# Gadersd/whisper-burn

Hardware: NVIDIA H100
Metric: audio-seconds/sec (higher is better)
Workload: dtype f32 (fp16-exact weights, fp32 activations/accumulate)

## Files before the change

whisper-burn_b200/csrc/decoder4.cu:

```cuda
#include <cooperative_groups.h>

#include "dec_common.cuh"

namespace cg = cooperative_groups;

namespace wb {

namespace {

#ifndef D4_ASYNC
#define D4_ASYNC 1
#endif
#define D4_EXCHANGE(IDX, RXBYTES, SEND, PF)                  \
    do {                                                     \
        WB_FINE();                                           \
        __syncthreads();                                     \
        WB_FINE();                                           \
        SEND();                                              \
        WB_FINE();                                           \
        if (D4_ASYNC) {                                      \
            PF();                                            \
            WB_FINE();                                       \
            xwait(xbar + (IDX), (RXBYTES), lc & 1u);         \
        } else {                                             \
            cluster_arrive();                                \
            PF();                                            \
            WB_FINE();                                       \
            cluster_wait();                                  \
        }                                                    \
    } while (0)
#ifndef D4_FINE
#define D4_FINE 0
#endif
#if D4_FINE
#define WB_FINE() WB_TRACE()
#else
#define WB_FINE() do { } while (0)
#endif

constexpr int CS = 16;
constexpr int LG_NBUF = 3;
constexpr int LG_RB = 8;
constexpr int KV_STG = 4;
#ifndef D4_L2_CKV_KEEP
#define D4_L2_CKV_KEEP 0
#endif
__device__ __forceinline__ uint64_t ckv_policy() { return D4_L2_CKV_KEEP ? l2_policy_evict_last() : l2_policy_evict_first(); }

__device__ __forceinline__ void cluster_arrive() { asm volatile("barrier.cluster.arrive.release.aligned;" ::: "memory"); }
__device__ __forceinline__ void cluster_wait() { asm volatile("barrier.cluster.wait.acquire.aligned;" ::: "memory"); }

template <int NR>
struct RowBias {
    float bias[NR];
    float bias_own;
};
template <int NR, int VPL>
struct RowRegs : RowBias<NR> {
    uint4 v[NR][VPL];
};

template <int NR>
__device__ __forceinline__ void load_bias(const float* __restrict__ bias, int row0, int step, RowBias<NR>& r) {
    const int lane = threadIdx.x & 31;
#pragma unroll
    for (int i = 0; i < NR; ++i) r.bias[i] = __ldg(bias + row0 + i * step);
    r.bias_own = __ldg(bias + row0 + min(lane >> 1, NR - 1) * step);
}
template <int NR, int VPL>
__device__ __forceinline__ void load_rows(const __half* __restrict__ W, const float* __restrict__ bias, int K, int row0, int step,
                                          RowRegs<NR, VPL>& r, uint64_t pol) {
    const int lane = threadIdx.x & 31, nv = K / 8;
    load_bias<NR>(bias, row0, step, r);
#pragma unroll
    for (int i = 0; i < NR; ++i) {
        const uint4* p = reinterpret_cast<const uint4*>(W + (int64_t)(row0 + i * step) * K);
#pragma unroll
        for (int j = 0; j < VPL; ++j) {
            const int v = j * 32 + lane;
            r.v[i][j] = v < nv ? ldg_l2(p + v, pol) : make_uint4(0, 0, 0, 0);
        }
    }
}
template <int NR>
__device__ __forceinline__ float warp_reduce_owner(const float (&acc)[NR]) {
    const int lane = threadIdx.x & 31;
    float v8[8], v4[4], v2[2];
    {
        const bool up = lane & 16;
#pragma unroll
        for (int i = 0; i < 8; ++i) {
            const float lo = i < NR ? acc[i] : 0.0f, hi = i + 8 < NR ? acc[i + 8] : 0.0f;
            const float recv = __shfl_xor_sync(0xffffffffu, up ? lo : hi, 16);
            v8[i] = (up ? hi : lo) + recv;
        }
    }
    {
        const bool up = lane & 8;
#pragma unroll
        for (int i = 0; i < 4; ++i) {
            const float recv = __shfl_xor_sync(0xffffffffu, up ? v8[i] : v8[i + 4], 8);
            v4[i] = (up ? v8[i + 4] : v8[i]) + recv;
        }
    }
    {
        const bool up = lane & 4;
#pragma unroll
        for (int i = 0; i < 2; ++i) {
            const float recv = __shfl_xor_sync(0xffffffffu, up ? v4[i] : v4[i + 2], 4);
            v2[i] = (up ? v4[i + 2] : v4[i]) + recv;
        }
    }
    const bool up = lane & 2;
    float v = (up ? v2[1] : v2[0]) + __shfl_xor_sync(0xffffffffu, up ? v2[0] : v2[1], 2);
    v += __shfl_xor_sync(0xffffffffu, v, 1);
    return v;
}

template <int NR, int VPL, bool REDUCE, typename WV>
__device__ __forceinline__ void dot_rows(WV&& wv, const float* xs, int K, float (&acc)[NR]) {
    const int lane = threadIdx.x & 31, nv = K / 8;
#pragma unroll
    for (int i = 0; i < NR; ++i) acc[i] = 0.0f;
#pragma unroll
    for (int j = 0; j < VPL; ++j) {
        const int v = j * 32 + lane;
        if (v < nv) {
            const float4 x0 = *reinterpret_cast<const float4*>(xs + v * 8);
            const float4 x1 = *reinterpret_cast<const float4*>(xs + v * 8 + 4);
#pragma unroll
            for (int i = 0; i < NR; ++i) {
                float w[8];
                cvt8(wv(i, j), w);
                float a = acc[i];
                a = fmaf(w[0], x0.x, a); a = fmaf(w[1], x0.y, a); a = fmaf(w[2], x0.z, a); a = fmaf(w[3], x0.w, a);
                a = fmaf(w[4], x1.x, a); a = fmaf(w[5], x1.y, a); a = fmaf(w[6], x1.z, a); a = fmaf(w[7], x1.w, a);
                acc[i] = a;
            }
        }
    }
    if constexpr (REDUCE) {
#pragma unroll
        for (int i = 0; i < NR; ++i) acc[i] = warp_sum(acc[i]);
    }
}
template <int NR, int VPL, bool REDUCE = true>
__device__ __forceinline__ void dot_rows1(const RowRegs<NR, VPL>& r, const float* xs, int K, float (&acc)[NR]) {
    dot_rows<NR, VPL, REDUCE>([&](int i, int j) { return r.v[i][j]; }, xs, K, acc);
}
template <int NR, int VPL, bool REDUCE = true>
__device__ __forceinline__ void dot_rows1s(const uint8_t* ws, const float* xs, int K, float (&acc)[NR]) {
    const int lane = threadIdx.x & 31, nv = K / 8;
    const uint4* w = reinterpret_cast<const uint4*>(ws) + (threadIdx.x >> 5) * nv;
    dot_rows<NR, VPL, REDUCE>([&](int i, int j) { return w[i * NW * nv + j * 32 + lane]; }, xs, K, acc);
}
__device__ __forceinline__ void bulk_rows(uint8_t* dst, const __half* W, int K, int row0, int n, uint64_t* bar) {
    const uint32_t bytes = (uint32_t)n * K * 2;
    fence_proxy_async();
    mbar_expect_tx(bar, bytes);
    bulk_g2s_l2(dst, W + (int64_t)row0 * K, bytes, bar, l2_policy_evict_last());
}

__device__ __forceinline__ void st_async_v4(uint32_t raddr, const float4& v, uint32_t rbar) {
    asm volatile("st.async.shared::cluster.mbarrier::complete_tx::bytes.v4.f32 [%0], {%1, %2, %3, %4}, [%5];" ::"r"(raddr), "f"(v.x),
                 "f"(v.y), "f"(v.z), "f"(v.w), "r"(rbar)
                 : "memory");
}
__device__ __forceinline__ void put16(cg::cluster_group& cl, float* dst, uint64_t* bar, int dest, const float4& v) {
#if D4_ASYNC
    st_async_v4(mapa_u32(smem_u32(dst), (uint32_t)dest), v, mapa_u32(smem_u32(bar), (uint32_t)dest));
#else
    *reinterpret_cast<float4*>(cl.map_shared_rank(dst, dest)) = v;
#endif
}
template <int CNT>
__device__ __forceinline__ void put_slice(cg::cluster_group& cl, const float* stage_s, float* dst_local, uint64_t* bar) {
    static_assert(CNT % 4 == 0, "slice must be a whole number of 16-byte vectors");
    constexpr int Q = CNT / 4;
    for (int i = threadIdx.x; i < CS * Q; i += NT) {
        const int dest = i / Q, q = i - dest * Q;
        put16(cl, dst_local + 4 * q, bar, dest, reinterpret_cast<const float4*>(stage_s)[q]);
    }
}
__device__ __forceinline__ void xwait(uint64_t* bar, uint32_t bytes, uint32_t parity) {
    if (threadIdx.x == 0) mbar_expect_tx(bar, bytes);
    const uint32_t mb = smem_u32(bar);
    uint32_t done = 0;
    int spins = 0;
    while (!done) {
        done = mbar_try_wait(mb, parity);
        if (!done && ++spins > (1 << 24)) __trap();
    }
}

template <int PF>
struct XRegs {
    float4 v[PF];
};
__device__ __forceinline__ float4 add4(const float4& a, const float4& b) {
    return make_float4(__fadd_rn(a.x, b.x), __fadd_rn(a.y, b.y), __fadd_rn(a.z, b.z), __fadd_rn(a.w, b.w));
}
template <int PF>
__device__ __forceinline__ void x_update(XRegs<PF>& x, const float* src_s, const float* d_s, float* dst_s) {
    const int lane = threadIdx.x & 31;
#pragma unroll
    for (int k = 0; k < PF; ++k)
        x.v[k] = add4(reinterpret_cast<const float4*>(src_s)[lane + 32 * k], reinterpret_cast<const float4*>(d_s)[lane + 32 * k]);
    if (dst_s != nullptr && threadIdx.x < 32) {
#pragma unroll
        for (int k = 0; k < PF; ++k) reinterpret_cast<float4*>(dst_s)[lane + 32 * k] = x.v[k];
    }
}
template <int D, int PF>
__device__ __forceinline__ void ln_fetch(float* lnp, const float* __restrict__ g, const float* __restrict__ b, uint64_t pol) {
    const int lane = threadIdx.x & 31;
#pragma unroll
    for (int k = 0; k < PF; ++k) {
        cp_async16_l2(lnp + 4 * (lane + 32 * k), g + 4 * (lane + 32 * k), pol);
        cp_async16_l2(lnp + D + 4 * (lane + 32 * k), b + 4 * (lane + 32 * k), pol);
    }
}
template <int D, int PF>
__device__ __forceinline__ void ln_warp(XRegs<PF>& x, const float* gb_s, float eps, int eps_outside, float* out_s) {
    const int lane = threadIdx.x & 31;
    cp_async_wait_all();
    float s = 0.0f;
#pragma unroll
    for (int k = 0; k < PF; ++k) s += (x.v[k].x + x.v[k].y) + (x.v[k].z + x.v[k].w);
    s = warp_sum(s);
    const float mean = __fdiv_rn(s, (float)D);
    float q = 0.0f;
#pragma unroll
    for (int k = 0; k < PF; ++k) {
        x.v[k].x = __fsub_rn(x.v[k].x, mean); x.v[k].y = __fsub_rn(x.v[k].y, mean);
        x.v[k].z = __fsub_rn(x.v[k].z, mean); x.v[k].w = __fsub_rn(x.v[k].w, mean);
        q = fmaf(x.v[k].x, x.v[k].x, q); q = fmaf(x.v[k].y, x.v[k].y, q);
        q = fmaf(x.v[k].z, x.v[k].z, q); q = fmaf(x.v[k].w, x.v[k].w, q);
    }
    q = warp_sum(q);
    const float var = __fdiv_rn(q, (float)D);
    const float den = eps_outside ? __fadd_rn(__fsqrt_rn(var), eps) : __fsqrt_rn(__fadd_rn(var, eps));
    const float rinv = __fdiv_rn(1.0f, den);
#pragma unroll
    for (int k = 0; k < PF; ++k) {
        const float4 g = reinterpret_cast<const float4*>(gb_s)[lane + 32 * k];
        const float4 b = reinterpret_cast<const float4*>(gb_s + D)[lane + 32 * k];
        reinterpret_cast<float4*>(out_s)[lane + 32 * k] =
            make_float4(fmaf(__fmul_rn(x.v[k].x, rinv), g.x, b.x), fmaf(__fmul_rn(x.v[k].y, rinv), g.y, b.y),
                        fmaf(__fmul_rn(x.v[k].z, rinv), g.z, b.z), fmaf(__fmul_rn(x.v[k].w, rinv), g.w, b.w));
    }
    __syncwarp();
}

template <int D, int RC, typename KVT>
__global__ void __launch_bounds__(NT, 1)
dec4_kernel(const DecArgs a) {
    extern __shared__ __align__(16) float sm[];
    cg::cluster_group cl = cg::this_cluster();
    constexpr int H = D / 64;
    constexpr int VPL = (D / 8 + 31) / 32;
    constexpr int VPL4 = (4 * D / 8 + 31) / 32;
    constexpr int NR_QKV = 3 * D / (CS * NW), NR_D = D / (CS * NW), NR_H = 4 * D / (CS * NW);
    const int L = a.L, V = a.V, R = a.R, t_max = a.t_max;
    const int tid = threadIdx.x, warp = tid >> 5, lane = tid & 31;
    const int rank = (int)cl.block_rank();
    const int row = blockIdx.x / CS;
    const bool active = row < R;

    float* lnp = sm + warp * 2 * D;
    float* qkv_s = sm + NW * 2 * D;
    float* att_s = qkv_s + 3 * D;
    float* dl_s = att_s + D;
    float* q2_s = dl_s + D;
    float* hid_s = q2_s + D;
    float* part_s = hid_s + 4 * D;
    float* wm = part_s + CS * 68;
    float* wl = wm + NW;
    float* wo = wl + NW;
    float* ao = wo + NW * 64;
    float* ML = ao + 64;
    constexpr int STG_N = 4 * D / CS > 68 ? 4 * D / CS : 68;
    float* stg_s = ML + 4;
    float* xb = stg_s + STG_N;
    float* xn_s = xb + 2 * D;
    float* red = xn_s + D;
    constexpr int RINGW = (LG_NBUF * LG_RB * D * 2 > KV_STG * 8 * 128 * 4) ? LG_NBUF * LG_RB * D * 2 : KV_STG * 8 * 128 * 4;
    constexpr int LG_PITCH = D * 2;
    uint8_t* ring = reinterpret_cast<uint8_t*>(red + NW * 4 * RC * 6);
    uint64_t* lg_bar = reinterpret_cast<uint64_t*>(ring + (size_t)NW * RINGW);
    uint64_t* kv_bar = lg_bar + NW * LG_NBUF;
    uint64_t* xbar = kv_bar + NW * KV_STG;
    uint64_t* wt_bar = xbar + 8;
    uint4* pl_hi = reinterpret_cast<uint4*>(wt_bar + 4);
    uint4* pl_lo = pl_hi + (D / 32) * 32;
    constexpr int QKV_B = 3 * D / CS * D * 2, W1_B = 4 * D / CS * D * 2, W2_B = D / CS * 4 * D * 2;
    constexpr int QKV_OFF = 0, W1_OFF = 0, W2_OFF = W1_OFF + W1_B;
    static_assert(W2_OFF + W2_B <= NW * RINGW, "W1 and W2 must fit the ring");
    static_assert(QKV_OFF + QKV_B <= W2_OFF, "the next layer's Wqkv arrives while W2 is read: no overlap");
    static_assert(QKV_B % 16 == 0 && W1_B % 16 == 0 && W2_B % 16 == 0 && W2_OFF % 16 == 0, "bulk copies move 16-byte units");
    if (lane == 0) {
        for (int j = 0; j < KV_STG; ++j) mbar_init(kv_bar + warp * KV_STG + j, 1);
        for (int j = 0; j < LG_NBUF; ++j) mbar_init(lg_bar + warp * LG_NBUF + j, 1);
        if (warp == 0) {
            for (int j = 0; j < 8; ++j) mbar_init(xbar + j, 1);
            for (int j = 0; j < 3; ++j) mbar_init(wt_bar + j, 1);
        }
        mbar_fence_init();
    }
    cl.sync();
    unsigned int lc = 0;
    unsigned int kv_count = 0;
    unsigned int lg_count = 0;
    unsigned int gen = 0;
    unsigned int lstep = 0;
    int tr_n = 0;
    const float scale = a.qk_scale;
    auto issue_qkv = [&](int l) {
        if (tid == 0) bulk_rows(ring + QKV_OFF, reinterpret_cast<const __half*>(a.layers[l].Wqkv), D, rank * (3 * D / CS), 3 * D / CS, wt_bar + 0);
    };
    auto demote = [&]() {
        const size_t gt = (size_t)blockIdx.x * NT + tid, gn = (size_t)gridDim.x * NT;
        for (int l = 0; l < L; ++l) {
            const DecLayer& W = a.layers[l];
            l2_demote(W.Wqkv, (size_t)3 * D * D * 2, gt, gn);
            l2_demote(W.Wo, (size_t)D * D * 2, gt, gn);
            l2_demote(W.Wcq, (size_t)D * D * 2, gt, gn);
            l2_demote(W.Wco, (size_t)D * D * 2, gt, gn);
            l2_demote(W.W1, (size_t)4 * D * D * 2, gt, gn);
            l2_demote(W.W2, (size_t)4 * D * D * 2, gt, gn);
            l2_demote(W.ln1_g, D * 4, gt, gn); l2_demote(W.ln1_b, D * 4, gt, gn); l2_demote(W.ln2_g, D * 4, gt, gn);
            l2_demote(W.ln2_b, D * 4, gt, gn); l2_demote(W.ln3_g, D * 4, gt, gn); l2_demote(W.ln3_b, D * 4, gt, gn);
        }
        l2_demote(a.lnf_g, D * 4, gt, gn);
        l2_demote(a.lnf_b, D * 4, gt, gn);
        const size_t kv_bytes = (size_t)L * a.Rmax * t_max * D * sizeof(KVT);
        l2_demote(a.kc, kv_bytes, gt, gn);
        l2_demote(a.vc, kv_bytes, gt, gn);
        if (D4_L2_CKV_KEEP) l2_demote(a.ckv, (size_t)L * a.Mcap * 2 * D * sizeof(KVT), gt, gn);
    };
    WB_TRACE();

    const __half* nullw = nullptr;
    (void)nullw;
    for (int step = 0; step < a.n_steps; ++step) {
        const int p = a.pos0 + step;
        const bool want_logits = p >= a.logits_from;
        constexpr int KH = D / 2, NCH = KH / 32;
        constexpr uint32_t BLKB = 16 * KH * 2;
        static_assert(LG_NBUF * LG_RB * D * 2 >= LG_NBUF * (int)BLKB, "ring slot too small");
        const __half* Et = reinterpret_cast<const __half*>(a.E_tiled);
        const int v_tiles = (V + 15) / 16;
        const int t0w = (int)blockIdx.x + (int)gridDim.x * warp, tstep = (int)gridDim.x * NW;
        const int my_tiles = t0w < v_tiles ? (v_tiles - t0w + tstep - 1) / tstep : 0;
        const int total = my_tiles * 2;
        auto tile_of = [&](int i) { return t0w + i * tstep; };
        uint8_t* wring = ring + (size_t)warp * RINGW;
        uint64_t* wbar = lg_bar + warp * LG_NBUF;
        auto issue = [&](int it) {
            if (it < total && lane == 0) {
                const int vt = tile_of(it >> 1);
                const int slot = (int)((lg_count + (unsigned int)it) % LG_NBUF);
                mbar_expect_tx(wbar + slot, BLKB);
                bulk_g2s_l2(wring + (size_t)slot * BLKB, Et + ((int64_t)vt * 2 + (it & 1)) * 16 * KH, BLKB, wbar + slot, l2_policy_evict_first());
            }
        };
        uint4* gpl_hi = reinterpret_cast<uint4*>(a.att_pl);
        uint4* gpl_lo = gpl_hi + (D / 32) * 32;
        if (want_logits && !active) {
#pragma unroll
            for (int j = 0; j < LG_NBUF; ++j) issue(j);
        }
        if (active) {
            const int tok = __ldcg(a.tokens + (int64_t)row * t_max + p);
            const int xh = rank % H, xci = rank / H;
            const int xnch = (CS - xh + H - 1) / H;
            const int xw = __ldcg(a.row_window + row);
            const int xT = a.win_T[xw];
            const int64_t xoff = a.win_row_off[xw] * (int64_t)(2 * D) + (int64_t)xh * xT * 128;
            const int sub = lane >> 2, l4 = lane & 3;
            const bool self_fast = p + 1 <= NW * 16;
            constexpr int PF = D / 128;
            static_assert(D % 128 == 0, "row must be a whole number of float4s per lane");
            int xsel = 0;
            XRegs<PF> x;
#pragma unroll
            for (int k = 0; k < PF; ++k)
                x.v[k] = add4(__ldg(reinterpret_cast<const float4*>(a.tok_emb + (int64_t)tok * D) + lane + 32 * k),
                              __ldg(reinterpret_cast<const float4*>(a.pos_emb + (int64_t)p * D) + lane + 32 * k));
            if (warp == 0) {
#pragma unroll
                for (int k = 0; k < PF; ++k) reinterpret_cast<float4*>(xb)[lane + 32 * k] = x.v[k];
            }
            RowBias<NR_QKV> b_qkv;
            load_bias<NR_QKV>(a.layers[0].bqkv, rank * (3 * D / CS) + warp, NW, b_qkv);
            if (step == 0) issue_qkv(0);
            if (step == 0) ln_fetch<D, PF>(lnp, a.layers[0].ln1_g, a.layers[0].ln1_b, l2_policy_evict_last());
            __syncthreads();
            for (int l = 0; l < L; ++l) {
                const DecLayer& W = a.layers[l];
                KVT* kcl = reinterpret_cast<KVT*>(a.kc) + (size_t)l * a.Rmax * t_max * D;
                KVT* vcl = reinterpret_cast<KVT*>(a.vc) + (size_t)l * a.Rmax * t_max * D;
                if (l > 0) {
                    x_update<PF>(x, xb + xsel * D, dl_s, xb + (xsel ^ 1) * D);
                    xsel ^= 1;
                }
                ln_warp<D, PF>(x, lnp, W.ln1_eps, a.eps_outside, xn_s);
                ln_fetch<D, PF>(lnp, W.ln2_g, W.ln2_b, l2_policy_evict_last());
                {
                    float acc[NR_QKV];
                    mbar_wait(wt_bar + 0, lc & 1u);
                    dot_rows1s<NR_QKV, VPL, false>(ring + QKV_OFF, xn_s, D, acc);
                    float mine = warp_reduce_owner<NR_QKV>(acc);
                    mine = __fadd_rn(mine, b_qkv.bias_own);
                    const int j = warp + (lane >> 1) * NW;
                    if (rank * (3 * D / CS) + j < 2 * D) mine = __fmul_rn(mine, scale);
                    if (!(lane & 1) && (lane >> 1) < NR_QKV) stg_s[j] = mine;
                }
                RowRegs<NR_D, VPL> w_o;
                constexpr int SNV = sizeof(KVT) == 4 ? 4 : 2;
                uint8_t* sring = ring + (size_t)warp * RINGW;
                auto pre_s2 = [&]() {
                    load_rows<NR_D, VPL>(reinterpret_cast<const __half*>(W.Wo), W.bo, D, rank * (D / CS) + warp, NW, w_o, l2_policy_evict_last());
                    if (rank < H && self_fast) {
#pragma unroll
                        for (int u = 0; u < 2; ++u) {
                            const int j = warp + NW * (u * 8 + sub);
                            if (j < p) {
                                const int64_t o = ((int64_t)row * t_max + j) * D + rank * 64 + l4 * 16;
#pragma unroll
                                for (int c = 0; c < SNV; ++c) {
                                    cp_async16_l2(sring + ((u * 2 + 0) * 4 + c) * 512 + lane * 16, reinterpret_cast<const uint4*>(kcl + o) + c, l2_policy_evict_last());
                                    cp_async16_l2(sring + ((u * 2 + 1) * 4 + c) * 512 + lane * 16, reinterpret_cast<const uint4*>(vcl + o) + c, l2_policy_evict_last());
                                }
                            }
                        }
                    }
                };
                auto send_s1 = [&]() {
                    put_slice<3 * D / CS>(cl, stg_s, qkv_s + rank * (3 * D / CS), xbar + 0);
                    if (tid < 3 * D / CS) {
                        const int n = rank * (3 * D / CS) + tid;
                        const float v = stg_s[tid];
                        if (n >= 2 * D) vcl[((int64_t)row * t_max + p) * D + (n - 2 * D)] = (KVT)v;
                        else if (n >= D) kcl[((int64_t)row * t_max + p) * D + (n - D)] = (KVT)v;
                    }
                };
                D4_EXCHANGE(0, 3 * D * 4, send_s1, pre_s2);
                if (D4_ASYNC && !self_fast) cl.sync();
                WB_TRACE();
                if (rank < H) {
                    const int h = rank;
                    if (self_fast) {
                        cp_async_wait_all();
                        float q[16];
#pragma unroll
                        for (int c = 0; c < 4; ++c) {
                            const float4 t4 = *reinterpret_cast<const float4*>(qkv_s + h * 64 + l4 * 16 + c * 4);
                            q[c * 4] = t4.x; q[c * 4 + 1] = t4.y; q[c * 4 + 2] = t4.z; q[c * 4 + 3] = t4.w;
                        }
                        AttnAcc A;
                        A.m = -INFINITY;
                        A.l = 0.0f;
#pragma unroll
                        for (int c = 0; c < 16; ++c) A.o[c] = 0.0f;
#pragma unroll
                        for (int u = 0; u < 2; ++u) {
                            const int j = warp + NW * (u * 8 + sub);
                            float4 skk[4], svv[4];
                            if (j < p) {
                                if constexpr (sizeof(KVT) == 4) {
#pragma unroll
                                    for (int c = 0; c < 4; ++c) {
                                        skk[c] = *reinterpret_cast<const float4*>(sring + ((u * 2 + 0) * 4 + c) * 512 + lane * 16);
                                        svv[c] = *reinterpret_cast<const float4*>(sring + ((u * 2 + 1) * 4 + c) * 512 + lane * 16);
                                    }
                                } else {
#pragma unroll
                                    for (int c = 0; c < 2; ++c) {
                                        float w8[8];
                                        cvt8(*reinterpret_cast<const uint4*>(sring + ((u * 2 + 0) * 4 + c) * 512 + lane * 16), w8);
                                        skk[2 * c] = make_float4(w8[0], w8[1], w8[2], w8[3]); skk[2 * c + 1] = make_float4(w8[4], w8[5], w8[6], w8[7]);
                                        cvt8(*reinterpret_cast<const uint4*>(sring + ((u * 2 + 1) * 4 + c) * 512 + lane * 16), w8);
                                        svv[2 * c] = make_float4(w8[0], w8[1], w8[2], w8[3]); svv[2 * c + 1] = make_float4(w8[4], w8[5], w8[6], w8[7]);
                                    }
                                }
                            } else {
#pragma unroll
                                for (int c = 0; c < 4; ++c) { skk[c] = make_float4(0.f, 0.f, 0.f, 0.f); svv[c] = skk[c]; }
                            }
                            if (j == p) {
#pragma unroll
                                for (int c = 0; c < 4; ++c) {
                                    float4 k4 = *reinterpret_cast<const float4*>(qkv_s + D + h * 64 + l4 * 16 + c * 4);
                                    float4 v4 = *reinterpret_cast<const float4*>(qkv_s + 2 * D + h * 64 + l4 * 16 + c * 4);
                                    if constexpr (sizeof(KVT) == 2) {
                                        k4 = make_float4((float)(KVT)k4.x, (float)(KVT)k4.y, (float)(KVT)k4.z, (float)(KVT)k4.w);
                                        v4 = make_float4((float)(KVT)v4.x, (float)(KVT)v4.y, (float)(KVT)v4.z, (float)(KVT)v4.w);
                                    }
                                    skk[c] = k4;
                                    svv[c] = v4;
                                }
                            }
                            attn_regs_step(q, skk, svv, j <= p, A);
                        }
                        attn_merge_subs(A);
                        attn_cta_tail(A, wm, wl, wo, ao, ML);
                    } else {
                        const KVT* kb = kcl + h * 64;
                        const KVT* vb = vcl + h * 64;
                        auto kp = [&](int j) { return kb + ((int64_t)row * t_max + j) * D; };
                        auto vp = [&](int j) { return vb + ((int64_t)row * t_max + j) * D; };
                        attn_cta(qkv_s + h * 64, p + 1, kp, vp, wm, wl, wo, ao, ML);
                    }
                }
                auto send_s2 = [&]() {
                    if (rank < H) {
                        const int dest = tid >> 4, q = tid & 15;
                        const float4 o4 = reinterpret_cast<const float4*>(ao)[q];
                        const float den = ML[1];
                        put16(cl, att_s + rank * 64 + 4 * q, xbar + 1, dest,
                              make_float4(__fdiv_rn(o4.x, den), __fdiv_rn(o4.y, den), __fdiv_rn(o4.z, den), __fdiv_rn(o4.w, den)));
                    }
                };
                auto pf_none = [&]() {};
                D4_EXCHANGE(1, D * 4, send_s2, pf_none);
                WB_TRACE();
                {
                    float acc[NR_D];
                    dot_rows1<NR_D, VPL>(w_o, att_s, D, acc);
                    WB_FINE();
                    if (lane == 0) {
#pragma unroll
                        for (int i = 0; i < NR_D; ++i) stg_s[warp + i * NW] = __fadd_rn(acc[i], w_o.bias[i]);
                    }
                }
                RowRegs<NR_D, VPL> w_cq;
                auto pre_s4 = [&]() {
                    load_rows<NR_D, VPL>(reinterpret_cast<const __half*>(W.Wcq), W.bcq, D, rank * (D / CS) + warp, NW, w_cq, l2_policy_evict_last());
                    fence_proxy_async();
                    attn_bulk_prefill<KV_STG, KVT, true>(reinterpret_cast<const KVT*>(a.ckv) + (size_t)l * a.Mcap * 2 * D + xoff, xT, xci * NW + warp,
                                                         xnch * NW, ring + (size_t)warp * RINGW, kv_bar + warp * KV_STG, kv_count, ckv_policy());
                };
                auto send_s3 = [&]() { put_slice<D / CS>(cl, stg_s, dl_s + rank * (D / CS), xbar + 2); };
                D4_EXCHANGE(2, D * 4, send_s3, pre_s4);
                WB_TRACE();
                x_update<PF>(x, xb + xsel * D, dl_s, xb + (xsel ^ 1) * D);
                xsel ^= 1;
                ln_warp<D, PF>(x, lnp, W.ln2_eps, a.eps_outside, xn_s);
                ln_fetch<D, PF>(lnp, W.ln3_g, W.ln3_b, l2_policy_evict_last());
                WB_FINE();
                {
                    float acc[NR_D];
                    dot_rows1<NR_D, VPL>(w_cq, xn_s, D, acc);
                    WB_FINE();
                    if (lane == 0) {
#pragma unroll
                        for (int i = 0; i < NR_D; ++i) stg_s[warp + i * NW] = __fmul_rn(__fadd_rn(acc[i], w_cq.bias[i]), scale);
                    }
                }
                RowRegs<NR_D, VPL> w_co;
                auto pre_s6 = [&]() { load_rows<NR_D, VPL>(reinterpret_cast<const __half*>(W.Wco), W.bco, D, rank * (D / CS) + warp, NW, w_co, l2_policy_evict_last()); };
                auto send_s4 = [&]() { put_slice<D / CS>(cl, stg_s, q2_s + rank * (D / CS), xbar + 3); };
                D4_EXCHANGE(3, D * 4, send_s4, pre_s6);
                WB_TRACE();
                {
                    const int h = xh, ci = xci, nch = xnch, T = xT;
                    const KVT* kbase = reinterpret_cast<const KVT*>(a.ckv) + (size_t)l * a.Mcap * 2 * D + xoff;
                    AttnAcc A;
                    attn_warp_bulk<KV_STG, KVT, true>(q2_s + h * 64, kbase, T, ci * NW + warp, nch * NW, 0, ring + (size_t)warp * RINGW,
                                                      kv_bar + warp * KV_STG, kv_count, A, true, ckv_policy());
                    if (lane < 4) {
#pragma unroll
                        for (int c = 0; c < 16; ++c) wo[warp * 64 + attn_bulk_dim<KVT>(lane, c)] = A.o[c];
                    }
                    if (lane == 0) { wm[warp] = A.m; wl[warp] = A.l; }
                    __syncthreads();
                    if (tid < 64) {
                        float M = -INFINITY;
#pragma unroll
                        for (int w2 = 0; w2 < NW; ++w2) M = fmaxf(M, wm[w2]);
                        float Ls = 0.0f, o = 0.0f;
#pragma unroll
                        for (int w2 = 0; w2 < NW; ++w2) {
                            const float m = wm[w2];
                            const float sc = m > -INFINITY ? expf(m - M) : 0.0f;
                            Ls += sc * wl[w2];
                            o += sc * wo[w2 * 64 + tid];
                        }
                        stg_s[4 + tid] = o;
                        if (tid < 4) stg_s[tid] = tid == 0 ? M : tid == 1 ? Ls : 0.0f;
                    }
                }
                auto send_s5 = [&]() { put_slice<68>(cl, stg_s, part_s + rank * 68, xbar + 4); };
                auto pre_mlp = [&]() {
                    if (tid == 0) {
                        bulk_rows(ring + W1_OFF, reinterpret_cast<const __half*>(W.W1), D, rank * (4 * D / CS), 4 * D / CS, wt_bar + 1);
                        bulk_rows(ring + W2_OFF, reinterpret_cast<const __half*>(W.W2), 4 * D, rank * (D / CS), D / CS, wt_bar + 2);
                    }
                };
                D4_EXCHANGE(4, CS * 68 * 4, send_s5, pre_mlp);
                WB_TRACE();
                for (int c = tid; c < D; c += NT) {
                    const int h = c / 64;
                    float M = -INFINITY;
                    for (int k = h; k < CS; k += H) M = fmaxf(M, part_s[k * 68]);
                    float den = 0.0f, num = 0.0f;
                    for (int k = h; k < CS; k += H) {
                        const float m = part_s[k * 68];
                        const float wgt = m > -INFINITY ? expf(m - M) : 0.0f;
                        den += wgt * part_s[k * 68 + 1];
                        num += wgt * part_s[k * 68 + 4 + (c & 63)];
                    }
                    att_s[c] = __fdiv_rn(num, den);
                }
                __syncthreads();
                {
                    float acc[NR_D];
                    dot_rows1<NR_D, VPL>(w_co, att_s, D, acc);
                    if (lane == 0) {
#pragma unroll
                        for (int i = 0; i < NR_D; ++i) stg_s[warp + i * NW] = __fadd_rn(acc[i], w_co.bias[i]);
                    }
                }
                RowBias<NR_H> b_1;
                auto pre_s7 = [&]() { load_bias<NR_H>(W.b1, rank * (4 * D / CS) + warp, NW, b_1); };
                auto send_s6 = [&]() { put_slice<D / CS>(cl, stg_s, dl_s + rank * (D / CS), xbar + 5); };
                D4_EXCHANGE(5, D * 4, send_s6, pre_s7);
                WB_TRACE();
                x_update<PF>(x, xb + xsel * D, dl_s, xb + (xsel ^ 1) * D);
                xsel ^= 1;
                ln_warp<D, PF>(x, lnp, W.ln3_eps, a.eps_outside, xn_s);
                if (l == L - 1 && want_logits && rank == 0 && warp == 0) {
                    ln_fetch<D, PF>(lnp, a.lnf_g, a.lnf_b, l2_policy_evict_last());
                } else {
                    const DecLayer& Wn = a.layers[l + 1 < L ? l + 1 : 0];
                    ln_fetch<D, PF>(lnp, Wn.ln1_g, Wn.ln1_b, l2_policy_evict_last());
                }
                WB_FINE();
                {
                    float acc[NR_H];
                    mbar_wait(wt_bar + 1, lc & 1u);
                    dot_rows1s<NR_H, VPL, false>(ring + W1_OFF, xn_s, D, acc);
                    float mine = warp_reduce_owner<NR_H>(acc);
                    mine = gelu_erf(__fadd_rn(mine, b_1.bias_own));
                    WB_FINE();
                    if (!(lane & 1) && (lane >> 1) < NR_H) stg_s[warp + (lane >> 1) * NW] = mine;
                }
                RowBias<NR_D> b_2;
                auto pre_s8 = [&]() {
                    load_bias<NR_D>(W.b2, rank * (D / CS) + warp, NW, b_2);
                    if (l + 1 < L) issue_qkv(l + 1);
                    else if (!want_logits && step + 1 < a.n_steps) issue_qkv(0);
                };
                auto send_s7 = [&]() { put_slice<4 * D / CS>(cl, stg_s, hid_s + rank * (4 * D / CS), xbar + 6); };
                D4_EXCHANGE(6, 4 * D * 4, send_s7, pre_s8);
                WB_TRACE();
                {
                    float acc[NR_D];
                    mbar_wait(wt_bar + 2, lc & 1u);
                    dot_rows1s<NR_D, VPL4>(ring + W2_OFF, hid_s, 4 * D, acc);
                    if (lane == 0) {
#pragma unroll
                        for (int i = 0; i < NR_D; ++i) stg_s[warp + i * NW] = __fadd_rn(acc[i], b_2.bias[i]);
                    }
                }
                auto pre_s1 = [&]() {
                    if (l + 1 < L) {
                        load_bias<NR_QKV>(a.layers[l + 1].bqkv, rank * (3 * D / CS) + warp, NW, b_qkv);
                    } else if (want_logits) {
                        fence_proxy_async();
#pragma unroll
                        for (int j = 0; j < LG_NBUF; ++j) issue(j);
                    }
                };
                auto send_s8 = [&]() { put_slice<D / CS>(cl, stg_s, dl_s + rank * (D / CS), xbar + 7); };
                D4_EXCHANGE(7, D * 4, send_s8, pre_s1);
                ++lc;
                WB_TRACE();
            }
            if (want_logits && rank == 0 && warp == 0) {
                x_update<PF>(x, xb + xsel * D, dl_s, nullptr);
                ln_warp<D, PF>(x, lnp, a.lnf_eps, a.eps_outside, xn_s);
#pragma unroll
                for (int k = 0; k < PF; ++k)
                    store_frag(gpl_hi, RC == 4 ? gpl_hi + 16 : gpl_lo, D / 32, row, 4 * (lane + 32 * k), reinterpret_cast<const float4*>(xn_s)[lane + 32 * k]);
                ln_fetch<D, PF>(lnp, a.layers[0].ln1_g, a.layers[0].ln1_b, l2_policy_evict_last());
            }
        }
        if (!want_logits) {
            if (D4_ASYNC && active) cl.sync();
            continue;
        }
        WB_TRACE();
        grid_sync(a.bar, gen);
        WB_TRACE();
        {
            const bool use_mask = SPECIAL_MASKED(a, p);
            const int eot_cap = a.loop_rules ? a.eot : -1;
            for (int i = tid; i < 2 * (D / 32) * 32; i += NT) cp_async16(pl_hi + i, gpl_hi + i);
            cp_async_wait_all();
            __syncthreads();
            WB_TRACE();
            const int g = lane >> 2, t = lane & 3;
            float m_run[2] = {-INFINITY, -INFINITY}, s_run[2] = {0.0f, 0.0f}, bv[2] = {-INFINITY, -INFINITY};
            int bi[2] = {INT_MAX, INT_MAX};
            float ah[4], al[4];
            unsigned int sp01 = 0;
#pragma unroll 1
            for (int it = 0; it < total; ++it) {
                const unsigned int cnt = lg_count + (unsigned int)it;
                const int slot = (int)(cnt % LG_NBUF);
                mbar_wait(wbar + slot, (cnt / LG_NBUF) & 1);
                const uint8_t* blk = wring + (size_t)slot * BLKB;
                const int half = it & 1;
                if (half == 0) {
#pragma unroll
                    for (int c = 0; c < 4; ++c) { ah[c] = 0.0f; al[c] = 0.0f; }
                    if (use_mask) {
                        const int n = tile_of(it >> 1) * 16 + g;
                        sp01 = (n < V ? ldg_l2(a.is_special + n, l2_policy_evict_first()) : 0u) | (n + 8 < V ? ldg_l2(a.is_special + n + 8, l2_policy_evict_first()) << 8 : 0u);
                    }
                }
#pragma unroll
                for (int c = 0; c < NCH; ++c) {
                    const uint4 a0 = *reinterpret_cast<const uint4*>(blk + (size_t)g * (KH * 2) + c * 64 + t * 16);
                    const uint4 a8 = *reinterpret_cast<const uint4*>(blk + (size_t)(g + 8) * (KH * 2) + c * 64 + t * 16);
                    const int chunk = half * NCH + c;
                    const uint4 bh = pl_hi[chunk * 32 + lane];
                    mma16816(ah, a0.x, a8.x, a0.y, a8.y, bh.x, bh.y);
                    mma16816(ah, a0.z, a8.z, a0.w, a8.w, bh.z, bh.w);
                    if constexpr (RC != 4) {
                        const uint4 bl = pl_lo[chunk * 32 + lane];
                        mma16816(al, a0.x, a8.x, a0.y, a8.y, bl.x, bl.y);
                        mma16816(al, a0.z, a8.z, a0.w, a8.w, bl.z, bl.w);
                    }
                }
                if (half == 1) {
                    const int n0 = tile_of(it >> 1) * 16;
#pragma unroll
                    for (int c = 0; c < 4; ++c) {
                        const int n = n0 + g + (c >> 1) * 8, e = c & 1;
                        if constexpr (RC == 4) al[c] = __shfl_xor_sync(0xffffffffu, ah[c], 2);
                        if (n < V && 2 * t + e < R) {
                            const float raw = hl_join(ah[c], al[c]);
                            const float v = (use_mask && ((sp01 >> ((c >> 1) * 8)) & 0xffu)) ? __fadd_rn(raw, -INFINITY) : raw;
                            if (v > -INFINITY) softmax_add(m_run[e], s_run[e], v);
                            if (cand_better(v, n, bv[e], bi[e])) { bv[e] = v; bi[e] = n; }
                            if (n == eot_cap) a.eot_logit[2 * t + e] = v;
                        }
                    }
                }
                __syncwarp();
                issue(it + LG_NBUF);
            }
            lg_count += (unsigned int)total;
            WB_TRACE();
#pragma unroll
            for (int e = 0; e < 2; ++e) {
#pragma unroll
                for (int off = 4; off < 32; off <<= 1) {
                    softmax_merge(m_run[e], s_run[e], __shfl_xor_sync(0xffffffffu, m_run[e], off), __shfl_xor_sync(0xffffffffu, s_run[e], off));
                    cand_xor(bv[e], bi[e], off);
                }
                if (g == 0) {
                    float* rec = red + (warp * 8 + 2 * t + e) * 4;
                    rec[0] = m_run[e]; rec[1] = s_run[e]; rec[2] = bv[e]; rec[3] = __int_as_float(bi[e]);
                }
            }
            __syncthreads();
            if (active && step + 1 < a.n_steps) issue_qkv(0);
            if (tid < R) fold_records_top1(a, red + tid * 4, NW, 8 * 4, (int64_t)blockIdx.x * R + tid);
        }
        WB_TRACE();
        ++lstep;
        __syncthreads();
        if (tid == 0) reinterpret_cast<int*>(ML)[2] = last_ticket(a.bar, lstep);
        __syncthreads();
        WB_TRACE();
        if (reinterpret_cast<int*>(ML)[2]) {
            __threadfence();
            for (int r = warp; r < R; r += NW) finish_row_top1<4>(a, r, p, gridDim.x);
            __syncthreads();
            if (tid == 0) release_flag(a.bar, lstep);
        }
        WB_TRACE();
        if (tid == 0) wait_flag(a.bar, lstep, 40000000000LL);
        __syncthreads();
        WB_TRACE();
        if (rows_open(a) == 0) {
            if (active && tid == 0 && step + 1 < a.n_steps) mbar_wait(wt_bar + 0, lc & 1u);
            if (blockIdx.x == 0 && tid == 0) decode_done(a, p + 1, 0, step + 1);
            demote();
            return;
        }
    }
    if (a.n_steps > 0 && a.pos0 + a.n_steps - 1 < a.logits_from) grid_sync(a.bar, gen);
    demote();
    if (blockIdx.x == 0 && tid == 0) decode_done(a, a.pos0 + a.n_steps, rows_open(a), a.n_steps);
}

template <int D, int RC>
constexpr size_t dec4_smem() {
    return sizeof(float) * ((size_t)(2 * NW + 13) * D + (4 * D / CS > 68 ? 4 * D / CS : 68) + CS * 68 + 2 * NW + NW * 64 + 64 + 4 + (size_t)NW * 4 * RC * 6 + 16) +
           (size_t)NW * std::max(LG_NBUF * LG_RB * D * 2, KV_STG * 8 * 128 * 4) + NW * LG_NBUF * 8 + NW * KV_STG * 8 + 8 * 8 + 4 * 8 + (size_t)2 * (D / 32) * 32 * 16 + 16;
}
static_assert(dec4_smem<384, 8>() <= 227 * 1024 && dec4_smem<384, 4>() <= 227 * 1024, "dec4_kernel exceeds the shared memory of an sm_90 CTA");

template <int D, int RC, typename KVT>
bool launch4_t(const DecArgs& a, cudaStream_t st) {
    const void* k = (const void*)dec4_kernel<D, RC, KVT>;
    const size_t smem = dec4_smem<D, RC>();
    static ClusterLaunch cl;
    const int n_cl = std::min(cl.capacity(k, CS, NT, smem, "dec4"), 8);
    if (n_cl < 1 || a.R > n_cl) return false;
    void* args[] = {(void*)&a};
    cl.launch(k, CS, n_cl, NT, smem, args, st, "dec4");
    return true;
}

}

bool launch_dec4(const DecArgs& a, bool w_half, cudaStream_t st) {
    if (!w_half || a.R > 8 || a.R < 1 || a.k != 1 || !a.greedy || a.use_cur_tok || a.anc != nullptr || a.logits_out != nullptr) return false;
    if (a.H * 64 != a.d || a.H > CS || a.E_tiled == nullptr) return false;
#define WB_D4(DD)                                                                                         \
    do {                                                                                                  \
        if (a.kv_half) return a.R <= 4 ? launch4_t<DD, 4, __half>(a, st) : launch4_t<DD, 8, __half>(a, st); \
        return a.R <= 4 ? launch4_t<DD, 4, float>(a, st) : launch4_t<DD, 8, float>(a, st);                 \
    } while (0)
    if (a.d == 384) WB_D4(384);
    if (a.d == 128) WB_D4(128);
#undef WB_D4
    return false;
}

}
```

Baseline: 2568.

## Keep vocab embedding tiles resident in shared memory of idle CTAs

CTAs without a decoding row now load a fixed slice of the tiled embedding matrix into their whole shared memory once per launch, using one bulk copy. The logits pass reads those resident tiles directly and streams only the remaining tiles through a smaller per-warp ring. This targets the per-step global/L2 traffic for the vocabulary projection. In exchange it reorganises the shared-memory layout, moves the ticket flag, and adds an extra mbarrier wait so the bulk copy has finished before the kernel exits.

```diff
diff --git a/whisper-burn_b200/csrc/decoder4.cu b/whisper-burn_b200/csrc/decoder4.cu
--- a/whisper-burn_b200/csrc/decoder4.cu
+++ b/whisper-burn_b200/csrc/decoder4.cu
@@ -41,6 +41,7 @@
 constexpr int CS = 16;
 constexpr int LG_NBUF = 3;
 constexpr int LG_RB = 8;
+constexpr int RL_NBUF = 2;
 constexpr int KV_STG = 4;
 #ifndef D4_L2_CKV_KEEP
 #define D4_L2_CKV_KEEP 0
@@ -251,6 +252,23 @@
     }
     __syncwarp();
 }
+
+template <int D, int RC>
+struct D4Smem {
+    static constexpr int STG_N = 4 * D / CS > 68 ? 4 * D / CS : 68;
+    static constexpr int RINGW = (LG_NBUF * LG_RB * D * 2 > KV_STG * 8 * 128 * 4) ? LG_NBUF * LG_RB * D * 2 : KV_STG * 8 * 128 * 4;
+    static constexpr int F_RING = (2 * NW + 13) * D + STG_N + CS * 68 + 2 * NW + NW * 64 + 64 + 4;
+    static constexpr size_t RES_CAP = (size_t)F_RING * 4 + (size_t)NW * RINGW;
+    static constexpr size_t RED_B = (size_t)NW * 4 * RC * 6 * 4;
+    static constexpr size_t BAR_B = (size_t)(NW * LG_NBUF + NW * KV_STG + 8 + 4) * 8;
+    static constexpr size_t PL_B = (size_t)2 * (D / 32) * 32 * 16;
+    static constexpr size_t BYTES = RES_CAP + RED_B + BAR_B + PL_B + 16;
+    static constexpr uint32_t BLKB = 16 * (D / 2) * 2;
+    static_assert(F_RING % 4 == 0 && RED_B % 16 == 0 && BAR_B % 16 == 0, "bulk-copy destinations are 16-byte aligned");
+    static constexpr int RES_T = (int)((RES_CAP - (size_t)NW * RL_NBUF * BLKB) / (2 * BLKB));
+    static_assert(RL_NBUF >= 1 && RL_NBUF <= LG_NBUF && RES_T >= 1, "a CTA without a row streams through its ring and holds resident tiles");
+    static_assert((size_t)RES_T * 2 * BLKB < (1u << 20), "one bulk copy completes at most 2^20 - 1 bytes on an mbarrier");
+};
 
 template <int D, int RC, typename KVT>
 __global__ void __launch_bounds__(NT, 1)
@@ -279,20 +297,23 @@
     float* wo = wl + NW;
     float* ao = wo + NW * 64;
     float* ML = ao + 64;
-    constexpr int STG_N = 4 * D / CS > 68 ? 4 * D / CS : 68;
+    using SM = D4Smem<D, RC>;
+    constexpr int STG_N = SM::STG_N, RINGW = SM::RINGW;
     float* stg_s = ML + 4;
     float* xb = stg_s + STG_N;
     float* xn_s = xb + 2 * D;
-    float* red = xn_s + D;
-    constexpr int RINGW = (LG_NBUF * LG_RB * D * 2 > KV_STG * 8 * 128 * 4) ? LG_NBUF * LG_RB * D * 2 : KV_STG * 8 * 128 * 4;
-    constexpr int LG_PITCH = D * 2;
-    uint8_t* ring = reinterpret_cast<uint8_t*>(red + NW * 4 * RC * 6);
-    uint64_t* lg_bar = reinterpret_cast<uint64_t*>(ring + (size_t)NW * RINGW);
+    uint8_t* ring = reinterpret_cast<uint8_t*>(sm + SM::F_RING);
+    uint8_t* res = reinterpret_cast<uint8_t*>(sm);
+    float* red = reinterpret_cast<float*>(res + SM::RES_CAP);
+    uint64_t* lg_bar = reinterpret_cast<uint64_t*>(red + NW * 4 * RC * 6);
     uint64_t* kv_bar = lg_bar + NW * LG_NBUF;
     uint64_t* xbar = kv_bar + NW * KV_STG;
     uint64_t* wt_bar = xbar + 8;
+    int* ticket = reinterpret_cast<int*>(wt_bar + 3);
     uint4* pl_hi = reinterpret_cast<uint4*>(wt_bar + 4);
     uint4* pl_lo = pl_hi + (D / 32) * 32;
+    static_assert(SM::RES_CAP == (size_t)SM::F_RING * 4 + (size_t)NW * RINGW && SM::RED_B == (size_t)NW * 4 * RC * 6 * 4,
+                  "the pointers above follow D4Smem");
     constexpr int QKV_B = 3 * D / CS * D * 2, W1_B = 4 * D / CS * D * 2, W2_B = D / CS * 4 * D * 2;
     constexpr int QKV_OFF = 0, W1_OFF = 0, W2_OFF = W1_OFF + W1_B;
     static_assert(W2_OFF + W2_B <= NW * RINGW, "W1 and W2 must fit the ring");
@@ -340,26 +361,36 @@
     };
     WB_TRACE();
 
+    constexpr int KH = D / 2, NCH = KH / 32;
+    constexpr uint32_t BLKB = SM::BLKB;
+    static_assert(LG_NBUF * LG_RB * D * 2 >= LG_NBUF * (int)BLKB, "ring slot too small");
+    const __half* Et = reinterpret_cast<const __half*>(a.E_tiled);
+    const int v_tiles = (V + 15) / 16;
+    const int n_act = CS * R;
+    const int res_all = min(v_tiles, ((int)gridDim.x - n_act) * SM::RES_T);
+    const int res0 = active ? 0 : ((int)blockIdx.x - n_act) * SM::RES_T;
+    const int my_res = active ? 0 : max(0, min(SM::RES_T, v_tiles - res0));
+    const int nbuf = active ? LG_NBUF : RL_NBUF;
+    if (!active && my_res > 0 && a.pos0 + a.n_steps > a.logits_from && tid == 0) {
+        mbar_expect_tx(xbar + 0, (uint32_t)my_res * 2 * BLKB);
+        bulk_g2s_l2(res, Et + (int64_t)res0 * 2 * 16 * KH, (uint32_t)my_res * 2 * BLKB, xbar + 0, l2_policy_evict_first());
+    }
+    const int t0w = res_all + (int)blockIdx.x + (int)gridDim.x * warp, tstep = (int)gridDim.x * NW;
+    const int my_tiles = t0w < v_tiles ? (v_tiles - t0w + tstep - 1) / tstep : 0;
+    const int stot = my_tiles * 2;
+    const int total = stot + 2 * (my_res > warp ? (my_res - warp + NW - 1) / NW : 0);
+    auto tile_of = [&](int i) { return i < my_tiles ? t0w + i * tstep : res0 + warp + (i - my_tiles) * NW; };
+    uint8_t* wring = active ? ring + (size_t)warp * RINGW : res + (size_t)SM::RES_T * 2 * BLKB + (size_t)warp * RL_NBUF * BLKB;
+    uint64_t* wbar = lg_bar + warp * LG_NBUF;
     const __half* nullw = nullptr;
     (void)nullw;
     for (int step = 0; step < a.n_steps; ++step) {
         const int p = a.pos0 + step;
         const bool want_logits = p >= a.logits_from;
-        constexpr int KH = D / 2, NCH = KH / 32;
-        constexpr uint32_t BLKB = 16 * KH * 2;
-        static_assert(LG_NBUF * LG_RB * D * 2 >= LG_NBUF * (int)BLKB, "ring slot too small");
-        const __half* Et = reinterpret_cast<const __half*>(a.E_tiled);
-        const int v_tiles = (V + 15) / 16;
-        const int t0w = (int)blockIdx.x + (int)gridDim.x * warp, tstep = (int)gridDim.x * NW;
-        const int my_tiles = t0w < v_tiles ? (v_tiles - t0w + tstep - 1) / tstep : 0;
-        const int total = my_tiles * 2;
-        auto tile_of = [&](int i) { return t0w + i * tstep; };
-        uint8_t* wring = ring + (size_t)warp * RINGW;
-        uint64_t* wbar = lg_bar + warp * LG_NBUF;
         auto issue = [&](int it) {
-            if (it < total && lane == 0) {
+            if (it < stot && lane == 0) {
                 const int vt = tile_of(it >> 1);
-                const int slot = (int)((lg_count + (unsigned int)it) % LG_NBUF);
+                const int slot = (int)((lg_count + (unsigned int)it) % (unsigned int)nbuf);
                 mbar_expect_tx(wbar + slot, BLKB);
                 bulk_g2s_l2(wring + (size_t)slot * BLKB, Et + ((int64_t)vt * 2 + (it & 1)) * 16 * KH, BLKB, wbar + slot, l2_policy_evict_first());
             }
@@ -367,8 +398,7 @@
         uint4* gpl_hi = reinterpret_cast<uint4*>(a.att_pl);
         uint4* gpl_lo = gpl_hi + (D / 32) * 32;
         if (want_logits && !active) {
-#pragma unroll
-            for (int j = 0; j < LG_NBUF; ++j) issue(j);
+            for (int j = 0; j < nbuf; ++j) issue(j);
         }
         if (active) {
             const int tok = __ldcg(a.tokens + (int64_t)row * t_max + p);
@@ -706,18 +736,25 @@
             int bi[2] = {INT_MAX, INT_MAX};
             float ah[4], al[4];
             unsigned int sp01 = 0;
+            if (total > stot) mbar_wait(xbar + 0, 0);
 #pragma unroll 1
             for (int it = 0; it < total; ++it) {
-                const unsigned int cnt = lg_count + (unsigned int)it;
-                const int slot = (int)(cnt % LG_NBUF);
-                mbar_wait(wbar + slot, (cnt / LG_NBUF) & 1);
-                const uint8_t* blk = wring + (size_t)slot * BLKB;
+                const int vt = tile_of(it >> 1);
+                const uint8_t* blk;
+                if (it < stot) {
+                    const unsigned int cnt = lg_count + (unsigned int)it;
+                    const int slot = (int)(cnt % (unsigned int)nbuf);
+                    mbar_wait(wbar + slot, (cnt / (unsigned int)nbuf) & 1);
+                    blk = wring + (size_t)slot * BLKB;
+                } else {
+                    blk = res + ((size_t)(vt - res0) * 2 + (it & 1)) * BLKB;
+                }
                 const int half = it & 1;
                 if (half == 0) {
 #pragma unroll
                     for (int c = 0; c < 4; ++c) { ah[c] = 0.0f; al[c] = 0.0f; }
                     if (use_mask) {
-                        const int n = tile_of(it >> 1) * 16 + g;
+                        const int n = vt * 16 + g;
                         sp01 = (n < V ? ldg_l2(a.is_special + n, l2_policy_evict_first()) : 0u) | (n + 8 < V ? ldg_l2(a.is_special + n + 8, l2_policy_evict_first()) << 8 : 0u);
                     }
                 }
@@ -736,7 +773,7 @@
                     }
                 }
                 if (half == 1) {
-                    const int n0 = tile_of(it >> 1) * 16;
+                    const int n0 = vt * 16;
 #pragma unroll
                     for (int c = 0; c < 4; ++c) {
                         const int n = n0 + g + (c >> 1) * 8, e = c & 1;
@@ -751,9 +788,9 @@
                     }
                 }
                 __syncwarp();
-                issue(it + LG_NBUF);
+                issue(it + nbuf);
             }
-            lg_count += (unsigned int)total;
+            lg_count += (unsigned int)stot;
             WB_TRACE();
 #pragma unroll
             for (int e = 0; e < 2; ++e) {
@@ -774,10 +811,10 @@
         WB_TRACE();
         ++lstep;
         __syncthreads();
-        if (tid == 0) reinterpret_cast<int*>(ML)[2] = last_ticket(a.bar, lstep);
+        if (tid == 0) *ticket = last_ticket(a.bar, lstep);
         __syncthreads();
         WB_TRACE();
-        if (reinterpret_cast<int*>(ML)[2]) {
+        if (*ticket) {
             __threadfence();
             for (int r = warp; r < R; r += NW) finish_row_top1<4>(a, r, p, gridDim.x);
             __syncthreads();
@@ -789,20 +826,21 @@
         WB_TRACE();
         if (rows_open(a) == 0) {
             if (active && tid == 0 && step + 1 < a.n_steps) mbar_wait(wt_bar + 0, lc & 1u);
+            if (!active && tid == 0 && my_res > 0) mbar_wait(xbar + 0, 0);
             if (blockIdx.x == 0 && tid == 0) decode_done(a, p + 1, 0, step + 1);
             demote();
             return;
         }
     }
     if (a.n_steps > 0 && a.pos0 + a.n_steps - 1 < a.logits_from) grid_sync(a.bar, gen);
+    if (!active && tid == 0 && my_res > 0 && a.pos0 + a.n_steps > a.logits_from) mbar_wait(xbar + 0, 0);
     demote();
     if (blockIdx.x == 0 && tid == 0) decode_done(a, a.pos0 + a.n_steps, rows_open(a), a.n_steps);
 }
 
 template <int D, int RC>
 constexpr size_t dec4_smem() {
-    return sizeof(float) * ((size_t)(2 * NW + 13) * D + (4 * D / CS > 68 ? 4 * D / CS : 68) + CS * 68 + 2 * NW + NW * 64 + 64 + 4 + (size_t)NW * 4 * RC * 6 + 16) +
-           (size_t)NW * std::max(LG_NBUF * LG_RB * D * 2, KV_STG * 8 * 128 * 4) + NW * LG_NBUF * 8 + NW * KV_STG * 8 + 8 * 8 + 4 * 8 + (size_t)2 * (D / 32) * 32 * 16 + 16;
+    return D4Smem<D, RC>::BYTES;
 }
 static_assert(dec4_smem<384, 8>() <= 227 * 1024 && dec4_smem<384, 4>() <= 227 * 1024, "dec4_kernel exceeds the shared memory of an sm_90 CTA");
 
```

Result: no change. 2607 (median of 6 runs) (+1.5%).
